# thomenr/Vent_Analysis

Measured on AMD Instinct MI355X. Metric: volumes/sec end-to-end VDP, 128×128×24 Xe volume, 1 GPU and 8-GPU batch, higher is better.
Workload: dtype f32; 1 GPU; batch of 256 synthetic 128x128x24 Xe volumes per GPU, end-to-end calculate_VDP: N4 (SimpleITK defaults 4x50 it) + mean-anchored + linear-binning + k-means VDP + defect border + SNR + cohort histogram; volumes_per_gpu=256, distinct_studies_per_gpu=192, lung_geometry=per study, parallelism=dp1, n4_subbatch=256, batches_in_flight=3

## Files before the change

vent_analysis_amd/csrc/n4.hip:

```cpp
#include <algorithm>
#include <cfloat>
#include <climits>
#include <cstring>

#include <hip/hip_cooperative_groups.h>

#include "n4_shared.h"

#define SEG_R 16
#define N4_CH 4096
#define N4_VPT (N4_CH / VH_TPB)
#define HIST_COPIES 8
#define FIT_WAVES 4
#ifndef FIT_GS
#define FIT_GS FIT_G
#endif
#ifndef FIT_WPE
#define FIT_WPE 1
#endif

float vh_bspline_eps(int max_spans) {
    float eps = 100.0f * FLT_EPSILON;
    while ((float)max_spans == (float)max_spans - eps) eps *= 10.0f;
    return eps;
// ... 1185 lines not shown
                                                   int64_t VS, int rsh, const float *T,
                                                   int64_t tbuf, int64_t tcap, DevLevel lv,
                                                   DevLevel lvo, int bo_mode, N4State *st,
                                                   double *part, int32_t c0, int conv_mode,
                                                   float *D) {
    extern __shared__ __attribute__((aligned(16))) float4 sW[];
    __shared__ double s_sd[VH_TPB / 64], s_sd2[VH_TPB / 64];
    __shared__ uint32_t s_max[VH_TPB / 64], s_min[VH_TPB / 64];
    const int32_t c = c0 + blockIdx.x;
    const int64_t b = cvol[c];
    if (!st[b].active) return;
    float4 *sWo = sW + R;
    int *sB = reinterpret_cast<int *>(sW + 2 * R);
    int *sBo = sB + R;
    const int ncx = lv.ax[0].ncp, ncxo = lvo.ax[0].ncp;
    for (int x = threadIdx.x; x < R; x += VH_TPB) {
        sW[x] = *reinterpret_cast<const float4 *>(lv.ax[0].w + 4 * x);
        sB[x] = lv.ax[0].base[x];
        sWo[x] = *reinterpret_cast<const float4 *>(lvo.ax[0].w + 4 * x);
        sBo[x] = lvo.ax[0].base[x];
    }
    const int64_t j0 = (int64_t)(c - cp[b]) * N4_CH;
    const int n = (int)(sc[b].n_mask1 - j0 < N4_CH ? sc[b].n_mask1 - j0 : N4_CH);
    const int64_t f = sc[b].first_masked;
    const int first = f < 0 ? -1 : (int)(((f / CZ) << rsh) | (f % CZ));
    const float *Lb = L0 + b * VS + j0;
    float *Ub = U + b * VS + j0;
    float *Db = D + b * VS + j0;
    const int32_t *Rb = ridx + b * VS + j0;
    const int tl = st[b].tlast;
    const __amdgpu_buffer_rsrc_t rTn = __builtin_amdgcn_make_buffer_rsrc(
        (void *)(T + (tl ^ 1) * tbuf + b * tcap), 0, (int)(tcap * 4), 0x00020000);
    const __amdgpu_buffer_rsrc_t rTo = __builtin_amdgcn_make_buffer_rsrc(
        (void *)(T + tl * tbuf + b * tcap), 0, (int)(tcap * 4), 0x00020000);
    int rr[N4_VPT];
    float la[N4_VPT];
#pragma unroll
    for (int k = 0; k < N4_VPT; ++k) {
        const int j = threadIdx.x + k * VH_TPB;
        const bool ok = j < n;
        rr[k] = ok ? Rb[j] : -1;
        la[k] = ok ? Lb[j] : 0.0f;
    }
    __syncthreads();
    double sd = 0.0, sd2 = 0.0;
    uint32_t kmax = 0u, kmin = 0xffffffffu;
    const int cmask = (1 << rsh) - 1;
#pragma unroll
    for (int h = 0; h < N4_VPT; h += 4) {
        float4 tn[4], to[4];
#pragma unroll
        for (int k = 0; k < 4; ++k) {
            const int r = rr[h + k];
            const int x = r < 0 ? 0 : r >> rsh;
            const int64_t col = r & cmask;
            const uint32_t on = r < 0 ? VH_OOB : (uint32_t)((col * ncx + sB[x]) * 4);
            const uint32_t oo = (r < 0 || !bo_mode) ? VH_OOB : (uint32_t)((col * ncxo + sBo[x]) * 4);
            const auto vn = __builtin_amdgcn_raw_buffer_load_b128(rTn, (int)on, 0, 0);
            const auto vo = __builtin_amdgcn_raw_buffer_load_b128(rTo, (int)oo, 0, 0);
            tn[k] = make_float4(__uint_as_float(vn[0]), __uint_as_float(vn[1]),
                                __uint_as_float(vn[2]), __uint_as_float(vn[3]));
            to[k] = make_float4(__uint_as_float(vo[0]), __uint_as_float(vo[1]),
                                __uint_as_float(vo[2]), __uint_as_float(vo[3]));
        }
#pragma unroll
        for (int k = 0; k < 4; ++k) {
            const int r = rr[h + k];
            if (r < 0) continue;
            const int x = r >> rsh;
            const int j = threadIdx.x + (h + k) * VH_TPB;
            const float4 w = sW[x], t = tn[k];
            const float bn = ((w.x * t.x + w.y * t.y) + w.z * t.z) + w.w * t.w;
            float bo = 0.0f;
            if (bo_mode) {
                const float4 wo = sWo[x], q = to[k];
                bo = ((wo.x * q.x + wo.y * q.y) + wo.z * q.z) + wo.w * q.w;
            }
            const float u = la[h + k] - bn;
            Ub[j] = u;
            if (conv_mode == 0) {
                Db[j] = bo - bn;
            } else {
                const double d = (double)expm1c(bo - bn);
                sd += d;
                sd2 = fma(d, d, sd2);
            }
            const uint32_t key = f2key(u);
            kmax = key > kmax ? key : kmax;
            if (r == first) st[b].u_first = u;
            else kmin = key < kmin ? key : kmin;
        }
    }
    for (int off = 32; off > 0; off >>= 1) {
        sd += __shfl_down(sd, off, 64);
        sd2 += __shfl_down(sd2, off, 64);
    }
    kmax = wave_max_u32(kmax);
    kmin = wave_min_u32(kmin);
    const int w = threadIdx.x >> 6;
    if ((threadIdx.x & 63) == 0) {
        s_sd[w] = sd;
        s_sd2[w] = sd2;
        s_max[w] = kmax;
        s_min[w] = kmin;
    }
    __syncthreads();
    if (threadIdx.x == 0) {
        double a = 0.0, a2 = 0.0;
        uint32_t mx = 0u, mn = 0xffffffffu;
        for (int i = 0; i < VH_TPB / 64; ++i) {
            a += s_sd[i];
            a2 += s_sd2[i];
            mx = s_max[i] > mx ? s_max[i] : mx;
            mn = s_min[i] < mn ? s_min[i] : mn;
        }
        part[(int64_t)c * 2] = a;
        part[(int64_t)c * 2 + 1] = a2;
        if (mx) atomicMax(&st[b].umax_key, mx);
        if (mn != 0xffffffffu) atomicMin(&st[b].umin_key, mn);
    }
}

#define WF_PROD 4
#define WF_TPB (64 * chain_waves(WF_PROD))
__global__ void __launch_bounds__(WF_TPB) k_n4_welford(const float *D, const int32_t *perm,
                                                                  int64_t VS, const VolScalars *sc,
                                                                  N4State *st, int64_t vol0) {
    __shared__ ChainSlot slots[CH_SLOTS];
    __shared__ ChainState cs;
    const int64_t b = vol0 + blockIdx.x;
    if (!st[b].active) return;
    chain_reset(slots, &cs);
    __syncthreads();
    const int64_t n = sc[b].n_mask1;
    const int w = threadIdx.x >> 6, pid = chain_prod_id(w);
    if (w == 0) chain_wave_mu(n, slots, &cs);
    else if (w == 1) chain_wave_sig(n, slots, &cs);
    else if (pid >= 0 && pid < WF_PROD)
        chain_wave_prod(D + b * VS, perm + b * VS, n, slots, &cs, pid, WF_PROD);
    __syncthreads();
    if (threadIdx.x == 0) st[b].conv_w = cs.conv;
}

__global__ void __launch_bounds__(PC_TPB) k_n4_pcw(const float *D, const int32_t *perm, float *Pbuf,
                                                   int64_t VS, const VolScalars *sc, N4State *st,
                                                   int64_t vol0, float skip_thresh) {
    extern __shared__ __attribute__((aligned(16))) char smem[];
    const int64_t b = vol0 + blockIdx.x;
    if (!st[b].active) return;
    PcShared<PC_TPB> &S = *reinterpret_cast<PcShared<PC_TPB> *>(smem);
    __shared__ ChainState ch;
    const float *const Db = D + b * VS;
    const int32_t *const pb = perm + b * VS;
    pcw_run<PC_TPB>([=](int64_t r) { return Db[pb[r]]; }, Pbuf + b * VS, sc[b].n_mask1, S, ch, 1,
            reinterpret_cast<double *>(const_cast<float *>(Db)), (int)(VS / 2), skip_thresh, nullptr,
            false, st[b].iters == 1 || st[b].pc_pre != 0);
    if (threadIdx.x == 0) {
        st[b].conv_w = ch.conv;
        st[b].pc_pre = S.xdone == 4 * 1 + 1;
        st[b].conv_bound = S.xdone == 4 * 1 + 1 || S.xdone == 4 * 1 + 3;
    }
}

struct PcgArgs {
    const float *D;
    const int32_t *perm;
    float *P;
    const VolScalars *sc;
    N4State *st;
    int64_t b;
    float *gmu, *gsig, *emu, *esig, *gmu_o, *emu_o;
    double *s1, *s2;
    double *agA, *agB, *agS;
    int *agF;
};
struct PcgLds {
    double wA[PC_TPB / 64], wB[PC_TPB / 64], wS[PC_TPB / 64];
    int wF[PC_TPB / 64];
    double pB, pS;
    int first;
};
__device__ void pcg_scan(const PcgArgs &A, PcgLds &L, cooperative_groups::grid_group &grid, double a,
                         double b, double bs, bool fail, double &dm, double &ds, int &first) {
    const int lane = threadIdx.x & 63, w = threadIdx.x >> 6, G = gridDim.x;
    const int NB = G * PC_TPB;
    double Aw = a, Bw = b, Sw = bs;
    for (int off = 1; off < 64; off <<= 1) {
        const double ya = __shfl_up(Aw, off, 64), yb = __shfl_up(Bw, off, 64), ys = __shfl_up(Sw, off, 64);
        if (lane >= off) {
            Bw = Aw * yb + Bw;
            Aw = Aw * ya;
            Sw = ys + Sw;
        }
    }
    const uint64_t bal = __ballot(fail);
    if (lane == 63) {
        L.wA[w] = Aw;
        L.wB[w] = Bw;
        L.wS[w] = Sw;
    }
    if (lane == 0) L.wF[w] = bal ? (int)(blockIdx.x * PC_TPB + w * 64 + __ffsll((unsigned long long)bal) - 1) : NB;
    double ea = __shfl_up(Aw, 1, 64), eb = __shfl_up(Bw, 1, 64), es = __shfl_up(Sw, 1, 64);
    if (lane == 0) {
        ea = 1.0;
        eb = 0.0;
        es = 0.0;
    }
    __syncthreads();
    if (threadIdx.x == 0) {
        double At = 1.0, Bt = 0.0, St = 0.0;
        int f = NB;
        for (int v = 0; v < PC_TPB / 64; ++v) {
            Bt = L.wA[v] * Bt + L.wB[v];
            At = At * L.wA[v];
            St = St + L.wS[v];
            f = min(f, L.wF[v]);
        }
        A.agA[blockIdx.x] = At;
        A.agB[blockIdx.x] = Bt;
        A.agS[blockIdx.x] = St;
        A.agF[blockIdx.x] = f;
    }
    grid.sync();
    if (w == 0) {
        double Al = 1.0, Bl = 0.0, Sl = 0.0;
        int f = NB;
        const int per = (G + 63) / 64;
        for (int i = 0; i < per; ++i) {
            const int u = per * lane + i;
            if (u < G) {
                f = min(f, A.agF[u]);
                if (u < (int)blockIdx.x) {
                    const double au = A.agA[u];
                    Bl = au * Bl + A.agB[u];
                    Al = Al * au;
                    Sl = Sl + A.agS[u];
                }
            }
        }
        for (int off = 1; off < 64; off <<= 1) {
            const double ya = __shfl_up(Al, off, 64), yb = __shfl_up(Bl, off, 64), ys = __shfl_up(Sl, off, 64);
            if (lane >= off) {
                Bl = Al * yb + Bl;
                Al = Al * ya;
                Sl = ys + Sl;
            }
            f = min(f, __shfl_xor(f, off, 64));
        }
        if (lane == 63) {
            L.pB = Bl;
            L.pS = Sl;
            L.first = f;
        }
    }
    __syncthreads();
    double x = L.pB, xs = L.pS;
    for (int v = 0; v < w; ++v) {
        x = L.wA[v] * x + L.wB[v];
        xs = xs + L.wS[v];
    }
    dm = ea * x + eb;
    ds = xs + es;
    first = L.first;
}

__global__ void __launch_bounds__(PC_TPB) k_n4_pcg(PcgArgs A) {
    namespace cg = cooperative_groups;
    cg::grid_group grid = cg::this_grid();
    if (!A.st[A.b].active) return;
    __shared__ PcgLds L;
    const int64_t n = A.sc[A.b].n_mask1;
    const int NB = gridDim.x * PC_TPB;
    const PcMap m = pc_map(n, NB);
    const uint32_t j = blockIdx.x * PC_TPB + threadIdx.x, len = pc_len(m, j), k0 = pc_k0(m, j);
    const int nbe = m.L ? NB : (int)m.rem;
    const float *const Db = A.D + A.b * 0;
    double s1 = 0.0, s2 = 0.0;
    for (uint32_t s0 = 0; s0 < len; s0 += 8) {
        int32_t pi[8];
#pragma unroll
        for (int i = 0; i < 8; ++i)
            pi[i] = A.perm[k0 - 1u + (s0 + i < len ? s0 + i : len - 1u)];
        float v[8];
#pragma unroll
        for (int i = 0; i < 8; ++i) v[i] = Db[pi[i]];
#pragma unroll
        for (int i = 0; i < 8; ++i)
            if (s0 + i < len) {
                const float p = expf_crs(v[i]);
                A.P[(size_t)(s0 + i) * NB + j] = p;
                const double e = (double)p - 1.0;
                s1 += e;
                s2 = fma(e, e, s2);
            }
    }
    double dm, ds;
    int first;
    pcg_scan(A, L, grid, 1.0, s1, s2, false, dm, ds, first);
    {
        const double K = (double)(k0 - 1u);
        float g = 0.0f, gs = 0.0f;
        if (K > 0.0) {
            g = (float)(1.0 + dm / K);
            const double v = ds - dm * (dm / K);
            gs = (float)(v > 0.0 ? v : 0.0);
        }
        A.gmu[j] = g;
// ... 592 lines not shown
```

vent_analysis_amd/csrc/n4_shared.h:

```cpp
#pragma once
#include "vh_internal.h"
#include "expf_small.h"
#include <cfloat>
#include <hip/hip_cooperative_groups.h>

struct DevAxis {
    const int32_t *base;
    const float *w;
    const double *sw2;
    const double *isw2;
    const double *w2;
    const double *w3;
    const double *w3i;
    const int2 *krange;
    int32_t n, ncp;
};
struct DevLevel {
    DevAxis ax[3];
    const int32_t *xst;
    const double *wk3;
    const double *wk2;
};

#define TILE_W 64
// ... 1236 lines not shown
            const double ulp = ldexp(1.0, e - 23), lim = ldexp(1.0, e + 1) - ulp;
            const double val = (double)s + (double)pre * ulp;
            const bool bad = in && lane >= from && (e < -125 || tie || big || !(val < lim));
            const uint64_t bb = __ballot(bad);
            if (!bb) {
                s = (float)__shfl(val, 63, 64);
                break;
            }
            const int f = (int)__builtin_ctzll(bb);
            const double before = f > from ? __shfl(val, f - 1, 64) : (double)s;
            const double tf = __shfl(t, f, 64);
            s = (float)((double)(float)before + tf);
            from = f + 1;
        }
    }
    return s;
}

template <int NL>
__device__ float pcx_walk_mu(const PcShared<NL> &S, const PcMap &m, const float *P, int j, float s) {
    const int lane = threadIdx.x & 63;
    const uint32_t len = pc_len(m, (uint32_t)j), k0 = pc_k0(m, (uint32_t)j);
    float mu = S.b[j].gmu;
    for (uint32_t s0 = 0; s0 < len; s0 += 64) {
        const bool in = s0 + lane < len;
        const float p = in ? P[(size_t)(s0 + lane) * NL + j] : 1.0f;
        const double kd = (double)(k0 + s0 + lane);
        const PcK q = pc_consts(kd, p);
        float mprev;
        mu = chain_sys64<true>(in ? q.A : 1.0, in ? q.B : 0.0, mu, mprev);
        double t = 0.0;
        if (in && kd != 1.0) {
            const float d = p - mprev;
            t = pc_div((double)(d * d) * (q.N - 1.0), q.N, q.r);
        }
        float rec;
        s = chain_sys64<false>(in ? 1.0 : 0.0, t, s, rec);
    }
    return s;
}

template <int NL>
__device__ bool pcx_scan(PcShared<NL> &S, const PcMap &m, const float *P, const double *tbuf, float &sig_out,
                         int &walks, int &slow) {
    const int lane = threadIdx.x & 63;
    const int nbe = m.L ? NL : (int)m.rem;
    bool bad = false;
    for (int j = lane; j < nbe - 1; j += 64)
        bad |= __float_as_uint(S.b[j].emu) != __float_as_uint(S.b[j + 1].gmu);
    if (__ballot(bad)) return false;
    float s = 0.0f;
    int j = 0;
    walks = slow = 0;
    int nxt = -1;
    double pf0 = 0.0, pf1 = 0.0;
    auto prefetch = [&](int from) {
        nxt = nbe;
        for (int c0 = from; c0 < nbe; c0 += 64) {
            const bool cnd = c0 + lane < nbe && (pcx_of(S, c0 + lane).flags & PCX_CANDF);
            const uint64_t bl = __ballot(cnd);
            if (bl) {
                nxt = c0 + (int)__builtin_ctzll(bl);
                break;
            }
        }
        if (nxt < nbe) {
            const PcX x = pcx_of(S, nxt);
            const uint32_t len = pc_len(m, (uint32_t)nxt);
            const double *tb = tbuf + (size_t)(x.slot >= 0 ? x.slot : 0) * (m.L + 1);
            pf0 = (x.slot >= 0 && (uint32_t)lane < len) ? tb[lane] : 0.0;
            pf1 = (x.slot >= 0 && (uint32_t)lane + 64 < len) ? tb[lane + 64] : 0.0;
        }
    };
    prefetch(0);
    while (j < nbe) {
        const int jj = j + lane;
        const bool have = jj < nbe;
        const int e = pcx_binade(s);
        bool ok = false;
        int inc = 0;
        if (have && e >= -125) {
            const PcX x = pcx_of(S, jj);
            ok = x.flags == 0 && x.e == e && x.c < (1 << 23);
            inc = ok ? x.c : 0;
        }
        const int pre = pcx_iscan(inc);
        const double ulp = ldexp(1.0, e - 23), lim = ldexp(1.0, e + 1) - ulp;
        const double end = (double)s + (double)pre * ulp;
        ok = ok && end < lim;
        const uint64_t fail = ~__ballot(ok || !have);
        const int first = fail ? (int)__builtin_ctzll(fail) : 64;
        if (first > 0) {
            const int last = min(first, nbe - j) - 1;
            s = (float)__shfl(end, last, 64);
            j += last + 1;
            continue;
        }
        const PcX x = pcx_of(S, j);
#ifdef PC_PROF
        const unsigned long long cw0 = clock64();
#endif
        if ((x.flags & PCX_CANDF) && x.slot >= 0) {
            const double a0 = j == nxt ? pf0 : 0.0, a1 = j == nxt ? pf1 : 0.0;
            const bool mine = j == nxt;
            if (mine) prefetch(j + 1);
            const double *tb = tbuf + (size_t)x.slot * (m.L + 1);
            const uint32_t len = pc_len(m, (uint32_t)j);
            s = mine ? pcx_walk_t(tb, len, s, a0, a1)
                     : pcx_walk_t(tb, len, s, (uint32_t)lane < len ? tb[lane] : 0.0,
                                  (uint32_t)lane + 64 < len ? tb[lane + 64] : 0.0);
        } else {
            s = pcx_walk_mu<NL>(S, m, P, j, s);
            ++slow;
        }
#ifdef PC_PROF
        if (lane == 0) S.xwcyc += clock64() - cw0;
#endif
        ++walks;
        ++j;
    }
    sig_out = s;
    return true;
}

#define PC_TPB 1024
#ifndef PC_APASS
#define PC_APASS 2
#endif
static_assert(PC_APASS >= 1 && PC_APASS <= 2, "PC_APASS: 1 or 2 phase-A stages (tag 2 is phase B's)");
#ifndef PC_AMAX
#define PC_AMAX 40
#endif
#ifndef PC_XSIG
#define PC_XSIG 1
#endif
#ifndef PC_G0
#define PC_G0 8
#endif
#ifndef PC_EXPS
#define PC_EXPS 1
#endif
#ifndef PC_S12F
#define PC_S12F 1
#endif
#ifndef PC_PRE
#define PC_PRE 1
#endif
#ifndef PC_P0CLAMP
#define PC_P0CLAMP 1
#endif
#ifndef PC_INLINE
#define PC_INLINE 0
#endif
template <int NL>
__host__ __device__ constexpr size_t pcw_lds_bytes() {
    return sizeof(PcShared<NL>) > sizeof(float) * PC_G0 * (NL + 8) ? sizeof(PcShared<NL>)
                                                                    : sizeof(float) * PC_G0 * (NL + 8);
}
#if PC_INLINE
#define PCW_INL __forceinline__
#else
#define PCW_INL __attribute__((noinline))
#endif
template <int NL, bool PEXP = false, class LoadD>
__device__ PCW_INL void pcw_run(LoadD ld, float *P, int64_t n, PcShared<NL> &S,
                                                  ChainState &ch, int req, double *tbuf, int tcap,
                                                  float skip_thresh = 0.0f, float *drift = nullptr,
                                                  bool drift_in = false, bool try_pre = false) {
    const int tid = threadIdx.x;
    const PcMap m = pc_map(n, NL);
    const uint32_t j = (uint32_t)tid, len = pc_len(m, j), k0 = pc_k0(m, j);
    const float dr = drift && drift_in ? drift[j] : 0.0f;
#ifdef PC_PROF
    const unsigned long long c0 = clock64();
    unsigned long long c1 = 0, c2 = 0;
    int ra = 0;
#endif
    constexpr int G0 = PC_G0, TS = NL + 8;
    static_assert(sizeof(float) * G0 * TS <= pcw_lds_bytes<NL>(), "pass-0 transpose buffer");
    float *const T0 = reinterpret_cast<float *>(&S);
    const uint32_t lmax = m.L + (m.rem ? 1u : 0u);
    double s1 = 0.0;
#if PC_S12F
    float s2 = 0.0f;
#else
    double s2 = 0.0;
#endif
    float pmax = -__int_as_float(0x7f800000), pmin = __int_as_float(0x7f800000);
    float v[G0];
    auto fetch = [&](uint32_t g0) {
#if PC_P0CLAMP
#pragma unroll
        for (int q = 0; q < G0; ++q) {
            const uint32_t jb = (uint32_t)tid / G0 + (uint32_t)(NL / G0) * q, i = (uint32_t)tid % G0;
            const uint32_t lb = pc_len(m, jb), ii = g0 + i;
            const int64_t r = lb ? (int64_t)(pc_k0(m, jb) - 1u + (ii < lb ? ii : lb - 1u)) : 0;
            v[q] = ld(r < n ? r : (n > 0 ? n - 1 : 0));
        }
#else
#pragma unroll
        for (int q = 0; q < G0; ++q) {
            const uint32_t jb = (uint32_t)tid / G0 + (uint32_t)(NL / G0) * q, i = (uint32_t)tid % G0;
            v[q] = g0 + i < pc_len(m, jb) ? ld((int64_t)(pc_k0(m, jb) - 1u + g0 + i)) : 0.0f;
        }
#endif
    };
    if (lmax) fetch(0);
#ifdef PC_PROF
    unsigned long long p0t[4] = {0, 0, 0, 0}, p0c = clock64();
#define P0M(k) do { const unsigned long long _c = clock64(); p0t[k] += _c - p0c; p0c = _c; } while (0)
#else
#define P0M(k) do { } while (0)
#endif
    for (uint32_t g0 = 0; g0 < lmax; g0 += G0) {
#pragma unroll
        for (int q = 0; q < G0; ++q)
            lds_st(T0 + (tid % G0) * TS + tid / G0 + (NL / G0) * q, v[q]);
        P0M(0);
        __syncthreads();
        P0M(1);
        if (g0 + G0 < lmax) fetch(g0 + G0);
        float tv[G0];
#pragma unroll
        for (int i = 0; i < G0; ++i) tv[i] = lds_ld(T0 + i * TS + j);
#pragma unroll
        for (int i = 0; i < G0; ++i)
            if (g0 + i < len) {
#ifdef AB_P0_FASTEXP
                const float p = PEXP ? tv[i] : __expf(tv[i]);
#else
                const float p = PEXP ? tv[i] : PC_EXPS ? expf_crs(tv[i]) : expf_cr(tv[i]);
#endif
                P[(size_t)(g0 + i) * NL + j] = p;
                s1 += (double)p - 1.0;
#if PC_S12F
                const float e = p - 1.0f;
                s2 = fmaf(e, e, s2);
#else
                const double e = (double)p - 1.0;
                s2 = fma(e, e, s2);
#endif
                pmax = fmaxf(pmax, p);
                pmin = fminf(pmin, p);
            }
        P0M(2);
        __syncthreads();
        P0M(3);
    }
#undef P0M
#ifdef PC_PROF
    if (blockIdx.x == 0 && tid == 0)
        printf("PCW_P0 loads %llu bar1 %llu work %llu bar2 %llu\n", p0t[0], p0t[1], p0t[2], p0t[3]);
#endif
    if (tid == 0) {
        S.done = 0;
        S.fallback = 0;
        S.xdone = 0;
        S.nfrz = 0;
        S.nfr = 0;
        S.xslots = 0;
    }
#ifdef PC_PROF
    if (tid < 32) S.pchg[tid] = S.pwav[tid] = 0;
#endif
    S.s1(j) = (double)s1;
    S.s2(j) = (double)s2;
    {
        const bool ok = k0 >= PC_FRZ_K0 && len > 0u;
        const double nd = itk_Nd((double)k0), nh1 = nd * PC_FRZ_H1, nh2 = nd * PC_FRZ_H2;
        const double fa1 = (double)pmax - nh1, fb1 = (double)pmin + nh1;
        const double fa2 = (double)pmax - nh2, fb2 = (double)pmin + nh2;
        const float inf = __int_as_float(0x7f800000);
        S.fz[j] = make_float4(ok && fa1 <= fb1 ? f_up(fa1) : inf, ok && fa1 <= fb1 ? f_dn(fb1) : -inf,
                              ok && fa2 <= fb2 ? f_up(fa2) : inf, ok && fa2 <= fb2 ? f_dn(fb2) : -inf);
    }
    __syncthreads();
    bool pre = false;
#if PC_PRE
    if (try_pre && skip_thresh > 0.0f && n > 1 && n < ((int64_t)1 << 24)) {
        double dmx, nbad;
        const bool okb = len == 0u || (pmax < 1.9f && pmin > 0.5f);
        if (len > 0u) atomicMax(&S.xslots, __float_as_int(pmax));
        pcw_scan<NL>(S, 1.0, S.s1(j), okb ? 0.0 : 1.0, dmx, nbad);
        const double Mx = (double)__int_as_float(S.xslots) * (1.0 + 0x1p-24 * ((double)n + 3.0)) * (1.0 + 0x1p-20);
        double Pk = dmx, acc = 0.0;
        const double cD = 0x1p-25 * Mx * (1.0 + 0x1p-20);
        for (uint32_t s0 = 0; s0 < len; s0 += 8) {
            float pv[8];
#pragma unroll
            for (int q = 0; q < 8; ++q) pv[q] = P[(size_t)(s0 + q < len ? s0 + q : len - 1u) * NL + j];
#pragma unroll
            for (int q = 0; q < 8; ++q) {
                const uint32_t k = k0 + s0 + (uint32_t)q;
                const double p = (double)pv[q];
                const bool in = s0 + (uint32_t)q < len;
                if (in && k >= 2u) {
                    const double r = (double)__frcp_rn((float)(k - 1u));
                    const double mk = fma(Pk, r, 1.0);
                    const double eps = fabs(mk - 1.0) * 0x1p-21 + 0x1p-50;
                    const double a = fabs(p - mk) - cD * (double)(k + 2u) - eps;
                    acc = a > 0.0 ? fma(a, a, acc) : acc;
                }
                Pk += in ? p - 1.0 : 0.0;
            }
        }
        const double wown = acc * (1.0 - 1.0 / fmax((double)k0, 2.0));
        double wpre, unused;
        __syncthreads();
        pcw_scan<NL>(S, 1.0, wown, 0.0, wpre, unused);
        if (tid == NL - 1) {
            const double f = pc_accum_factor((double)n + 8.0);
            const double lo = (wpre + wown) * f;
            const bool allok = nbad + (okb ? 0.0 : 1.0) == 0.0;
            float sl = (float)lo;
            if ((double)sl > lo && sl > 0.0f) sl = __uint_as_float(__float_as_uint(sl) - 1u);
            const double Pn = dmx + s1;
            const double mn = 1.0 + Pn / (double)n;
            const float muh = f_up(mn + cD * ((double)n + 3.0) + fabs(mn - 1.0) * 0x1p-50 + 0x1p-50);
            if (allok && lo > 0.0 && itk_conv(muh, sl, n) > skip_thresh) {
                S.mu = muh;
                S.sig = sl;
                S.rounds = 0;
                S.xdone = 4 * req + 1;
            }
        }
        __syncthreads();
        pre = S.xdone == 4 * req + 1;
    }
#endif
    double gd = 0.0;
    if (!pre) pcw_guess<NL>(S, m, gd, dr);
    __syncthreads();
#ifdef PC_PROF
    c1 = clock64();
#endif
    int round = 0;
#ifdef PC_PROF
    unsigned long long cblk = 0, cst[2] = {0, 0}, cbs[2] = {0, 0};
    int rst[2] = {0, 0};
#endif
    bool xs = pre;
    for (int pass = 0; pass < PC_APASS && !pre; ++pass) {
        if (pass == 1 && PC_XSIG && S.done == 4 * req) {
#ifdef PC_PROF
            const unsigned long long cx0 = clock64();
#endif
            const bool real = j < (uint32_t)(m.L ? NL : m.rem);
            const double own = real ? (double)S.b[j].esig : 0.0;
            const double wown = (real && k0 > 1u) ? own * (1.0 - 1.0 / fmin((double)k0, ITK_NMAX)) : 0.0;
            double sest, wpre;
            pcw_scan<NL>(S, 1.0, own, wown, sest, wpre);
            if (tid == NL - 1 && skip_thresh > 0.0f) {
                const double f = pc_accum_factor((double)n + (double)m.L + 8.0);
                const double lo = (wpre + wown) * f;
                float sl = (float)lo;
                if ((double)sl > lo && sl > 0.0f) sl = __uint_as_float(__float_as_uint(sl) - 1u);
                const int nbe = m.L ? NL : (int)m.rem;
                const float mue = S.b[nbe - 1].emu;
                const float muh = __uint_as_float(__float_as_uint(mue) + 1u);
                if (lo > 0.0 && mue > 0.0f && itk_conv(muh, sl, n) > skip_thresh) {
                    S.mu = mue;
                    S.sig = sl;
                    S.rounds = round + 1;
                    S.xdone = 4 * req + 3;
                }
            }
            if (tid == 0) S.xslots = 0;
            __syncthreads();
            if (S.xdone == 4 * req + 3) {
                xs = true;
                break;
            }
#ifdef PC_PROF
            const unsigned long long cxt = clock64();
#endif
            pcx_tpass<NL>(S, m, P, j, len, k0, sest, sest + own, tbuf, tcap);
            __syncthreads();
#ifdef PC_PROF
            cbs[1] = clock64() - cxt;
#endif
            if (tid < 64) {
#ifdef PC_PROF
                if (tid == 0) S.xwcyc = 0;
                const unsigned long long csc = clock64();
#endif
                float sg = 0.0f;
                int w = 0, slow = 0;
                const bool ok = pcx_scan<NL>(S, m, P, tbuf, sg, w, slow);
                if (tid == 0) {
                    const int nbe = m.L ? NL : (int)m.rem;
                    if (ok) {
                        S.mu = S.b[nbe - 1].emu;
                        S.sig = sg;
                        S.rounds = round + 1;
                        S.xdone = 4 * req + 3;
                    }
                    S.xwalks = ok ? w : -1;
                    S.xslow = slow;
#ifdef PC_PROF
                    S.xscyc = clock64() - csc;
#endif
                }
            }
            __syncthreads();
#ifdef PC_PROF
            cst[1] = clock64() - cx0;
#endif
            if (S.xdone == 4 * req + 3) {
                xs = true;
                break;
            }
        }
#ifdef PC_PROF
        const unsigned long long cs0 = clock64(), cb0 = cblk;
#endif
        const int tag = 4 * req + pass;
        float lg = __int_as_float(0x7fc00000), ls = lg, le = 0.0f, les = 0.0f;
        int amax = pass == 0 ? PC_AMAX0 : PC_AMAX;
        bool frz = false;
        for (int ra0 = 0; ra0 < amax; ++ra0, ++round) {
#ifdef PC_PROF
            const unsigned long long cq = clock64();
#endif
            const float g = lget(S.b[j].gmu), gs = lget(S.b[j].gsig);
            const bool same = __float_as_uint(g) == __float_as_uint(lg) && __float_as_uint(gs) == __float_as_uint(ls);
#ifdef PC_PROF
            if (pass == 0 && ra0 < 32 && (tid & 63) == 0) {
                const uint64_t bq = __ballot(!same);
                atomicAdd(&S.pchg[ra0], __popcll(bq));
                atomicAdd(&S.pwav[ra0], bq != 0ull);
            }
#endif
            if (__ballot(!same) != 0ull && !same) {
                float mu = g, sig = gs;
                if (pass == 0) pc_block_apx<NL, false>(P, j, len, k0, mu, sig, NL, (m.L + 1u) * NL);
                else pc_block_apx<NL, true>(P, j, len, k0, mu, sig, NL, (m.L + 1u) * NL);
                lg = g;
                ls = gs;
                le = mu;
                les = sig;
            }
            lset(S.b[j].emu, le);
            lset(S.b[j].esig, les);
            __syncthreads();
#ifdef PC_PROF
            cblk += clock64() - cq;
#endif
            pcw_update<NL>(S, m, round, tag, ra0 == amax - 1, pass == 0 && !frz, pass == 1);
            __syncthreads();
#ifdef PC_PROF
            rst[pass]++;
#endif
            if (S.done == tag) break;
            if (pass == 0 && !frz && S.fallback == tag) {
                frz = true;
                if (tid < 64) {
                    const bool all = pc_mu_serial_frozen<NL>(S, m, P);
                    if (tid == 0) {
                        S.nfr = all ? 1 : 0;
                        S.nfrz += all ? 1 : 100;
                    }
                }
                __syncthreads();
                if (S.nfr) amax = ra0 + 2;
            }
        }
#ifdef PC_PROF
        cst[pass] = clock64() - cs0;
        cbs[pass] = cblk - cb0;
#endif
    }
#ifdef PC_PROF
    ra = round + 1;
    c2 = clock64();
#endif
    const int tagb = 4 * req + 2;
    for (int rb = 0; rb < PC_RMAX && !xs; ++rb) {
        ++round;
        float mu = S.b[j].gmu, sig = S.b[j].gsig;
        pc_block<NL>(P, j, len, k0, mu, sig);
        S.b[j].emu = mu;
        S.b[j].esig = sig;
        __syncthreads();
        pcw_update<NL>(S, m, round, tagb, rb == PC_RMAX - 1, true);
        __syncthreads();
        if (S.done == tagb) break;
        if (S.fallback == tagb) {
            if (tid == 0) pc_serial<NL>(S, m, P);
            __syncthreads();
            break;
        }
    }
    if (drift && !pre && (xs || !drift_in)) drift[j] = xs ? (float)((double)S.b[j].gmu - gd) : 0.0f;
    if (drift && pre && !drift_in) drift[j] = 0.0f;
    if (tid == 0) {
        ch.mu = S.mu;
        ch.conv = itk_conv(S.mu, S.sig, n);
#ifdef PC_PROF
        if (blockIdx.x == 0)
            printf("PCW_PROF n %lld roundsA %d roundsB %d fallback %d pass0 %llu A %llu (blocks %llu) B %llu"
                   " | stage0 %d rounds %llu cyc (blocks %llu) stage1 %d rounds %llu cyc (blocks %llu) xsig %d walks %d\n",
                   (long long)n, ra, S.rounds - ra + 0, S.fallback == tagb, c1 - c0, c2 - c1, cblk, clock64() - c2,
                   rst[0], cst[0], cbs[0], rst[1], cst[1], cbs[1], (int)xs, S.xwalks * 1000 + S.xslow);
        if (blockIdx.x == 0)
            for (int r = 0; r < rst[0] && r < 32; ++r) printf("PCW_RND %d chg %d waves %d\n", r, S.pchg[r], S.pwav[r]);
        if (blockIdx.x == 0 && xs) printf("PCW_X scan %llu walks %llu\n", S.xscyc, S.xwcyc);
#endif
    }
}


template <int NS = CH_SLOTS>
__device__ void chain_wave_mu(int64_t n, ChainSlot *slots, ChainState *cs) {
    const int lane = threadIdx.x & 63;
    const int64_t nblk = (n + 63) / 64;
    unsigned long long wt = 0;
    __builtin_amdgcn_s_setprio(CH_PRIO);
    CH_T0();
    float muf = 0.0f;
    for (int64_t blk = 0; blk < nblk; ++blk) {
        ChainSlot &S = slots[blk % NS];
        CH_WAIT(wt, while (lds_load_acq(&S.ready) != (int)(blk + 1)) __builtin_amdgcn_s_sleep(1));
        const double2 q = S.ab[lane];
        float rec;
        muf = chain_sys64<true>(q.x, q.y, muf, rec);
        S.mu[lane] = rec;
        wave_lds_order();
        if (lane == 0) {
            if (blk == nblk - 1) cs->mu = muf;
            lds_store_rel(&cs->a_done, (int)(blk + 1));
        }
    }
    CH_DONE(0, wt);
    __builtin_amdgcn_s_setprio(0);
}

template <int NS = CH_SLOTS>
__device__ void chain_wave_sig(int64_t n, ChainSlot *slots, ChainState *cs) {
    const int lane = threadIdx.x & 63;
    float sig = 0.0f;
    const int64_t nblk = (n + 63) / 64;
    unsigned long long wt = 0;
    __builtin_amdgcn_s_setprio(CH_PRIO);
    CH_T0();
    for (int64_t blk = 0; blk < nblk; ++blk) {
        ChainSlot &S = slots[blk % NS];
        const int64_t j = blk * 64 + lane;
        CH_WAIT(wt, while (lds_load_acq(&cs->a_done) <= (int)blk) __builtin_amdgcn_s_sleep(1));
        const float q = S.p[lane] - S.mu[lane];
        const double N = S.nd[lane];
        const double t = ((double)(q * q) * (N - 1.0)) / N;
        const bool ok = j < n && j > 0;
        float rec;
        sig = chain_sys64<false>(ok ? 1.0 : 0.0, ok ? t : 0.0, sig, rec);
        (void)rec;
        wave_lds_order();
        if (lane == 0) lds_store_rel(&cs->b_done, (int)(blk + 1));
    }
    CH_DONE(1, wt);
    __builtin_amdgcn_s_setprio(0);
    if (lane == 0) {
        while (lds_load_acq(&cs->a_done) < (int)nblk) __builtin_amdgcn_s_sleep(1);
        cs->conv = itk_conv(cs->mu, sig, n);
    }
}

struct PcgWg {
    double A, B, S;
    float gfirst, gsfirst;
    float elast, eslast;
    int F;
    float enbe;
};
struct Pcg2Args {
    const float *D;
    const int32_t *perm;
    float *P;
    const VolScalars *sc;
    N4State *st;
    int64_t b;
    PcgWg *wg;
    float *E;
    float skip_thresh;
    unsigned long long *gran;
    uint32_t tag0;
    int32_t t0;
    unsigned long long *kst;
};
#define PCG_GW 12
__device__ __forceinline__ void pcg_publish(unsigned long long *g, const PcgWg &r, uint32_t tag) {
    const uint64_t a = (uint64_t)__double_as_longlong(r.A), bb = (uint64_t)__double_as_longlong(r.B),
                   s = (uint64_t)__double_as_longlong(r.S);
    const uint32_t v[PCG_GW] = {(uint32_t)a, (uint32_t)(a >> 32), (uint32_t)bb, (uint32_t)(bb >> 32),
                                (uint32_t)s, (uint32_t)(s >> 32), __float_as_uint(r.gfirst),
                                __float_as_uint(r.gsfirst), __float_as_uint(r.elast),
                                __float_as_uint(r.eslast), (uint32_t)r.F, __float_as_uint(r.enbe)};
#pragma unroll
    for (int k = 0; k < PCG_GW; ++k)
        __hip_atomic_store(g + k, ((unsigned long long)tag << 32) | v[k], __ATOMIC_RELAXED,
                           __HIP_MEMORY_SCOPE_AGENT);
}
__device__ __forceinline__ bool pcg_fetch(const unsigned long long *g, uint32_t tag, PcgWg &r) {
    uint32_t v[PCG_GW];
    bool ok = true;
#pragma unroll
    for (int k = 0; k < PCG_GW; ++k) {
        const unsigned long long x = __hip_atomic_load(g + k, __ATOMIC_RELAXED, __HIP_MEMORY_SCOPE_AGENT);
        ok &= (uint32_t)(x >> 32) == tag;
        v[k] = (uint32_t)x;
    }
    r.A = __longlong_as_double((long long)(((uint64_t)v[1] << 32) | v[0]));
    r.B = __longlong_as_double((long long)(((uint64_t)v[3] << 32) | v[2]));
    r.S = __longlong_as_double((long long)(((uint64_t)v[5] << 32) | v[4]));
    r.gfirst = __uint_as_float(v[6]);
    r.gsfirst = __uint_as_float(v[7]);
    r.elast = __uint_as_float(v[8]);
    r.eslast = __uint_as_float(v[9]);
    r.F = (int)v[10];
    r.enbe = __uint_as_float(v[11]);
    return ok;
}
struct Pcg2Lds {
    double wA[PC_TPB / 64], wB[PC_TPB / 64], wS[PC_TPB / 64];
    int wF[PC_TPB / 64];
    float gg[PC_TPB], gsg[PC_TPB];
    float elast, eslast, enbe;
    double pB, pS, tot;
    float mue;
    int first;
    double xA[PC_TPB / 64], xB[PC_TPB / 64], xS[PC_TPB / 64];
};
__device__ void pcg2_scan(const Pcg2Args &A, Pcg2Lds &L, cooperative_groups::grid_group &grid, int parity,
                          int nbe, double a, double b, double bs, bool mm, float g, float gs, float e, float es,
                          bool sum_mode, double &dm, double &ds, int &first, uint32_t tag = 0u) {
    const int t = threadIdx.x, lane = t & 63, w = t >> 6, G = gridDim.x;
    const int NB = G * PC_TPB;
    const bool last = t == PC_TPB - 1;
    if (t == 0) lset(L.enbe, 0.0f);
    __syncthreads();
    if ((int)(blockIdx.x * PC_TPB + t) == nbe - 1) lset(L.enbe, e);
    if (last) {
        b = 0.0;
        if (!sum_mode) bs = 0.0;
        mm = false;
        lset(L.elast, e);
        lset(L.eslast, es);
    }
    double Aw = a, Bw = b, Sw = bs;
    aff_step<0x111, 0xf>(Aw, Bw, Sw);
    aff_step<0x112, 0xf>(Aw, Bw, Sw);
    aff_step<0x114, 0xf>(Aw, Bw, Sw);
    aff_step<0x118, 0xf>(Aw, Bw, Sw);
    aff_step<0x142, 0xa>(Aw, Bw, Sw);
    aff_step<0x143, 0xc>(Aw, Bw, Sw);
    const uint64_t bal = __ballot(mm);
    if (lane == 63) {
        lset(L.wA[w], Aw);
        lset(L.wB[w], Bw);
        lset(L.wS[w], Sw);
    }
    if (lane == 0) lset(L.wF[w], bal ? (int)(blockIdx.x * PC_TPB + w * 64 + __ffsll((unsigned long long)bal) - 1) : NB);
// ... 345 lines not shown
```

Baseline: 17440 volumes/s.

## Make pass-0 transpose per-wave with wave barriers and split gather loads

Restructures the pass-0 LDS transpose in pcw_run so each wavefront owns its own tile covering its 64 columns. The two block-wide __syncthreads per iteration become wavefront-scoped fences and barriers, and each wave loops only over its own length. The permuted gather is split into an index-load phase and a value-load phase, separated by a sched_barrier, so the loads can overlap. Per-lane row bounds are also precomputed out of the loop. The change removes block-level synchronisation stalls in the hot pass, at the cost of more LDS for the per-wave tiles and a reliance on the per-wave length being uniform.

```diff
diff --git a/vent_analysis_amd/csrc/n4.hip b/vent_analysis_amd/csrc/n4.hip
--- a/vent_analysis_amd/csrc/n4.hip
+++ b/vent_analysis_amd/csrc/n4.hip
@@ -1361,7 +1361,7 @@
     __shared__ ChainState ch;
     const float *const Db = D + b * VS;
     const int32_t *const pb = perm + b * VS;
-    pcw_run<PC_TPB>([=](int64_t r) { return Db[pb[r]]; }, Pbuf + b * VS, sc[b].n_mask1, S, ch, 1,
+    pcw_run<PC_TPB>(PcPermLoad{Db, pb}, Pbuf + b * VS, sc[b].n_mask1, S, ch, 1,
             reinterpret_cast<double *>(const_cast<float *>(Db)), (int)(VS / 2), skip_thresh, nullptr,
             false, st[b].iters == 1 || st[b].pc_pre != 0);
     if (threadIdx.x == 0) {
diff --git a/vent_analysis_amd/csrc/n4_shared.h b/vent_analysis_amd/csrc/n4_shared.h
--- a/vent_analysis_amd/csrc/n4_shared.h
+++ b/vent_analysis_amd/csrc/n4_shared.h
@@ -1412,10 +1412,27 @@
 #ifndef PC_INLINE
 #define PC_INLINE 0
 #endif
+struct PcPermLoad {
+    const float *D;
+    const int32_t *perm;
+    __device__ __forceinline__ int32_t index(int64_t r) const { return perm[r]; }
+    __device__ __forceinline__ float value(int32_t i) const { return D[i]; }
+    __device__ __forceinline__ float operator()(int64_t r) const { return D[perm[r]]; }
+};
+template <class L>
+__device__ __forceinline__ auto pc_ld_index(const L &ld, int64_t r, int) -> decltype(ld.index(r)) { return ld.index(r); }
+template <class L>
+__device__ __forceinline__ int64_t pc_ld_index(const L &, int64_t r, long) { return r; }
+template <class L, class I>
+__device__ __forceinline__ auto pc_ld_value(const L &ld, I i, int) -> decltype(ld.value(i)) { return ld.value(i); }
+template <class L, class I>
+__device__ __forceinline__ float pc_ld_value(const L &ld, I r, long) { return ld(r); }
+#define PC_P0W (64 + 8)
 template <int NL>
 __host__ __device__ constexpr size_t pcw_lds_bytes() {
-    return sizeof(PcShared<NL>) > sizeof(float) * PC_G0 * (NL + 8) ? sizeof(PcShared<NL>)
-                                                                    : sizeof(float) * PC_G0 * (NL + 8);
+    return sizeof(PcShared<NL>) > sizeof(float) * PC_G0 * PC_P0W * (NL / 64)
+               ? sizeof(PcShared<NL>)
+               : sizeof(float) * PC_G0 * PC_P0W * (NL / 64);
 }
 #if PC_INLINE
 #define PCW_INL __forceinline__
@@ -1436,10 +1453,12 @@
     unsigned long long c1 = 0, c2 = 0;
     int ra = 0;
 #endif
-    constexpr int G0 = PC_G0, TS = NL + 8;
-    static_assert(sizeof(float) * G0 * TS <= pcw_lds_bytes<NL>(), "pass-0 transpose buffer");
-    float *const T0 = reinterpret_cast<float *>(&S);
-    const uint32_t lmax = m.L + (m.rem ? 1u : 0u);
+    constexpr int G0 = PC_G0, TS = PC_P0W, BQ = 64 / G0;
+    static_assert(64 % G0 == 0 && NL % 64 == 0, "pass 0: G0 lanes per block, whole waves");
+    static_assert(sizeof(float) * G0 * TS * (NL / 64) <= pcw_lds_bytes<NL>(), "pass-0 transpose tiles");
+    const uint32_t lane = (uint32_t)tid & 63u, wv = (uint32_t)__builtin_amdgcn_readfirstlane(tid >> 6);
+    float *const T0 = reinterpret_cast<float *>(&S) + wv * (uint32_t)(G0 * TS);
+    const uint32_t lmax = (uint32_t)__builtin_amdgcn_readfirstlane((int)pc_len(m, 64u * wv));
     double s1 = 0.0;
 #if PC_S12F
     float s2 = 0.0f;
@@ -1447,42 +1466,56 @@
     double s2 = 0.0;
 #endif
     float pmax = -__int_as_float(0x7f800000), pmin = __int_as_float(0x7f800000);
+    const uint32_t li = lane % G0;
+    uint32_t rb[G0], re[G0];
+#pragma unroll
+    for (int q = 0; q < G0; ++q) {
+        const uint32_t jb = 64u * wv + lane / G0 + (uint32_t)BQ * q, lb = pc_len(m, jb);
+        const int64_t last = lb ? (int64_t)(pc_k0(m, jb) - 1u + (lb - 1u)) : 0;
+        rb[q] = lb ? pc_k0(m, jb) - 1u + li : 0u;
+        re[q] = (uint32_t)(last < n ? last : (n > 0 ? n - 1 : 0));
+    }
     float v[G0];
     auto fetch = [&](uint32_t g0) {
 #if PC_P0CLAMP
+        decltype(pc_ld_index(ld, (int64_t)0, 0)) ix[G0];
 #pragma unroll
         for (int q = 0; q < G0; ++q) {
-            const uint32_t jb = (uint32_t)tid / G0 + (uint32_t)(NL / G0) * q, i = (uint32_t)tid % G0;
-            const uint32_t lb = pc_len(m, jb), ii = g0 + i;
-            const int64_t r = lb ? (int64_t)(pc_k0(m, jb) - 1u + (ii < lb ? ii : lb - 1u)) : 0;
-            v[q] = ld(r < n ? r : (n > 0 ? n - 1 : 0));
-        }
+            const uint32_t r = rb[q] + g0;
+            ix[q] = pc_ld_index(ld, (int64_t)(r < re[q] ? r : re[q]), 0);
+        }
+        __builtin_amdgcn_sched_barrier(0);
+#pragma unroll
+        for (int q = 0; q < G0; ++q) v[q] = pc_ld_value(ld, ix[q], 0);
 #else
 #pragma unroll
         for (int q = 0; q < G0; ++q) {
-            const uint32_t jb = (uint32_t)tid / G0 + (uint32_t)(NL / G0) * q, i = (uint32_t)tid % G0;
-            v[q] = g0 + i < pc_len(m, jb) ? ld((int64_t)(pc_k0(m, jb) - 1u + g0 + i)) : 0.0f;
+            const uint32_t jb = 64u * wv + lane / G0 + (uint32_t)BQ * q;
+            v[q] = g0 + li < pc_len(m, jb) ? ld((int64_t)(pc_k0(m, jb) - 1u + g0 + li)) : 0.0f;
         }
 #endif
     };
     if (lmax) fetch(0);
 #ifdef PC_PROF
-    unsigned long long p0t[4] = {0, 0, 0, 0}, p0c = clock64();
+    unsigned long long p0t[3] = {0, 0, 0}, p0c = clock64();
 #define P0M(k) do { const unsigned long long _c = clock64(); p0t[k] += _c - p0c; p0c = _c; } while (0)
 #else
 #define P0M(k) do { } while (0)
 #endif
     for (uint32_t g0 = 0; g0 < lmax; g0 += G0) {
 #pragma unroll
-        for (int q = 0; q < G0; ++q)
-            lds_st(T0 + (tid % G0) * TS + tid / G0 + (NL / G0) * q, v[q]);
+        for (int q = 0; q < G0; ++q) lds_st(T0 + li * TS + lane / G0 + BQ * q, v[q]);
+        __builtin_amdgcn_fence(__ATOMIC_RELEASE, "wavefront");
+        __builtin_amdgcn_wave_barrier();
+        __builtin_amdgcn_fence(__ATOMIC_ACQUIRE, "wavefront");
         P0M(0);
-        __syncthreads();
-        P0M(1);
         if (g0 + G0 < lmax) fetch(g0 + G0);
         float tv[G0];
 #pragma unroll
-        for (int i = 0; i < G0; ++i) tv[i] = lds_ld(T0 + i * TS + j);
+        for (int i = 0; i < G0; ++i) tv[i] = lds_ld(T0 + i * TS + lane);
+        __builtin_amdgcn_fence(__ATOMIC_RELEASE, "wavefront");
+        __builtin_amdgcn_wave_barrier();
+        __builtin_amdgcn_fence(__ATOMIC_ACQUIRE, "wavefront");
 #pragma unroll
         for (int i = 0; i < G0; ++i)
             if (g0 + i < len) {
@@ -1503,15 +1536,11 @@
                 pmax = fmaxf(pmax, p);
                 pmin = fminf(pmin, p);
             }
-        P0M(2);
-        __syncthreads();
-        P0M(3);
-    }
+        P0M(1);
+    }
+    __syncthreads();
+    P0M(2);
 #undef P0M
-#ifdef PC_PROF
-    if (blockIdx.x == 0 && tid == 0)
-        printf("PCW_P0 loads %llu bar1 %llu work %llu bar2 %llu\n", p0t[0], p0t[1], p0t[2], p0t[3]);
-#endif
     if (tid == 0) {
         S.done = 0;
         S.fallback = 0;
@@ -1522,6 +1551,7 @@
     }
 #ifdef PC_PROF
     if (tid < 32) S.pchg[tid] = S.pwav[tid] = 0;
+    if (tid == 0) S.xwcyc = S.xscyc = 0;
 #endif
     S.s1(j) = (double)s1;
     S.s2(j) = (double)s2;
@@ -1767,6 +1797,10 @@
         if (blockIdx.x == 0 && xs) printf("PCW_X scan %llu walks %llu\n", S.xscyc, S.xwcyc);
 #endif
     }
+#ifdef PC_PROF
+    if (blockIdx.x == 0 && lane == 0 && (wv == 0 || wv == NL / 64 - 1))
+        printf("PCW_P0 wave %u loads %llu work %llu bar %llu\n", wv, p0t[0], p0t[1], p0t[2]);
+#endif
 }
 
 
```

Result: faster. 17740 volumes/s (median of 6 runs) (+1.7%).
